# yeyupiaoling/MASR

Measured on AMD Instinct MI355X. Metric: audio-seconds/sec (RTF^-1), conformer_streaming_fbank b32x10s, PCM->fbank->encoder->ctc_greedy->text, higher is better.
Workload: dtype f32; 1 GPU; configs[1]: conformer.yml streaming fbank, batch=32 synthetic 16 kHz 10 s utterances per GPU, ctc_greedy, random-init weights V=4233; global_batch=32, parallelism=dp1, world_size_observed=1, backend=none

## Files before the change

### masr_amd/_lib.py

```python
import collections
import contextlib
import ctypes as C
import os

import numpy as _np

from .build import LIB_PATH

_lib = None


class MasrConfig(C.Structure):
    _fields_ = [('model_kind', C.c_int32), ('d_model', C.c_int32), ('heads', C.c_int32), ('d_ff', C.c_int32),
                ('num_blocks', C.c_int32), ('cnn_kernel', C.c_int32), ('n_mels', C.c_int32),
                ('vocab_size', C.c_int32), ('causal', C.c_int32), ('max_pos', C.c_int32), ('device_id', C.c_int32),
                ('reserved', C.c_int32 * 5)]


class MasrError(RuntimeError):
    pass


_P = C.c_void_p
_I = C.c_int32
# ... 115 lines not shown

def lib():
    global _lib
    if _lib is not None:
        return _lib
    import torch
    if not os.path.exists(LIB_PATH):
        raise MasrError(f'{LIB_PATH} not found: build it with `python -m masr_amd.build` '
                        f'(hipcc --offload-arch=gfx950). There is no CPU fallback.')
    h = C.CDLL(LIB_PATH)
    for name, args in SIGNATURES.items():
        fn = getattr(h, name)
        fn.argtypes = args
        fn.restype = _RESTYPE.get(name, C.c_int)
    _lib = h
    return h


def check(rc):
    if rc != 0:
        raise MasrError(lib().masr_last_error().decode('utf-8', 'replace'))


_ENGINE_KEYS = {'beam_profile': 2, 'prof_stride': 16, 'skip_padding': 38}


def debug_key_table():
    rows = []
    key, default, experimental, name = _I(), _I(), _I(), C.c_char_p()
    while lib().masr_debug_key_info(len(rows), C.byref(key), C.byref(default), C.byref(experimental), C.byref(name)) == 0:
        rows.append((key.value, name.value.decode(), default.value, bool(experimental.value)))
    return rows


FFN_KERNELS = ('X3', 'COOP', 'DUAL', 'ROWS16', 'PC')
FfnPlan = collections.namedtuple('FfnPlan', 'kernel nsplit cpb ny packed tail_in_kernel head_in_kernel split_head prof')


def ffn_plan(d_ff, M, keys=None, d_model=256, affine=0, tail_n=0, tail_planar=0, head_ktaps=0, head_norm=0):
    ask = (_I * 5)(affine, tail_n, tail_planar, head_ktaps, head_norm)
    flat = [int(v) for kv in (keys or {}).items() for v in kv]
    out = (_I * 9)()
    check(lib().masr_ffn_plan(d_model, d_ff, M, ask, (_I * max(1, len(flat)))(*flat), len(flat) // 2, out))
    return FfnPlan(FFN_KERNELS[out[0]], *out[1:])


@contextlib.contextmanager
# ... 11 lines not shown
```

### masr_amd/csrc/common.h

```cpp
#pragma once
#include <hip/hip_runtime.h>
#include <stdint.h>

#include "knobs.h"
#include "lm_scorer.h"

struct masr_resample_feed;
struct masr_resample_rate;

#ifndef MASR_EXPERIMENTS
#define MASR_EXPERIMENTS 0
#endif

typedef float f32x4 __attribute__((ext_vector_type(4)));
typedef float f32x16 __attribute__((ext_vector_type(16)));

namespace masr {

struct LdsAttr {
    size_t granted[32] = {};
};
void ensure_dynamic_lds(const void* fn, size_t bytes, LdsAttr& st);
void note_launch_error(const char* what, hipError_t e);

// ... 87 lines not shown
    const float *feats, *mean, *istd, *c1w, *c1b;
    int Tin, Fin;
};

void launch_gemm(const GemmArgs& a, int amode, int epi, hipStream_t s);
void launch_pack_conv2_rows(const float* w, float* p, int K, hipStream_t s);
bool gemm_conv2_rows(const GemmArgs& a);
void launch_gemm_splitk(const GemmArgs& a, float* partial, int nsplit, hipStream_t s, int amode = A_PLAIN);
struct FfnArgs;
#if MASR_EXPERIMENTS
bool launch_gemm_bf16x3(const GemmArgs& a, int amode, hipStream_t s);
size_t ffn_x3_packed_elems(int dff);
void launch_pack_ffn_x3(const float* w1, const float* w2, unsigned short* p1, unsigned short* p2, int dff, hipStream_t s);
bool launch_ffn_x3(const FfnArgs& a, hipStream_t s);
#else
inline bool launch_gemm_bf16x3(const GemmArgs&, int, hipStream_t) { return false; }
inline size_t ffn_x3_packed_elems(int) { return 0; }
inline void launch_pack_ffn_x3(const float*, const float*, unsigned short*, unsigned short*, int, hipStream_t) {}
inline bool launch_ffn_x3(const FfnArgs&, hipStream_t) { return false; }
#endif

void launch_layernorm(const float* x, const float* w, const float* b, float* y, int M, float eps,
                      int seq_t, int pad, const int* lens, hipStream_t s);
void launch_conv1(const float* feats, const float* mean, const float* istd, const float* w9c, const float* bias,
                  float* out, int B, int T, int F, int C, hipStream_t s);
bool launch_dwconv_ln_silu(const float* g, const float* wkc, const float* bias, const float* lnw, const float* lnb,
                           float* out, int nseq, int Tq, int ktaps, float eps, hipStream_t s, const float* gconst = nullptr);
void launch_glu_const(const float* bias512, float* out256, hipStream_t s);
void launch_queue_spin(long long ticks, hipStream_t s);
void launch_queue_nop(hipStream_t s);
bool launch_dwconv_bn_silu(const float* g, const float* wkc, const float* bias, const float* scale, const float* shift,
                           float* out, int nseq, int Tq, int ktaps, hipStream_t s, const float* gconst = nullptr);
void launch_dwconv_stride2_ln_silu(const float* g, const float* wkc, const float* bias, const float* lnw,
                                   const float* lnb, float* out, int nseq, int Tin, int ktaps, float eps, hipStream_t s);
void launch_dwconv_stride2_bn_silu(const float* g, const float* wkc, const float* bias, const float* scale,
                                   const float* shift, float* out, int nseq, int Tin, int ktaps, hipStream_t s);
void launch_avgpool2(const float* x, float* out, int B, int T, hipStream_t s);
void launch_time_reduce_dw(const float* x, const float* w5c, const float* bias, const int* lens, float* out, int B, int T,
                           int mstride, hipStream_t s);
void launch_recover_add(const float* saved, const float* y, float* x, int B, int T, int L, hipStream_t s);
void launch_softmax_argmax(float* logits, int M, int V, int ldv, int write_probs, int* idx, float* maxp, hipStream_t s);
void launch_ctc_collapse(const int* idx, const float* maxp, const int* nframes, int B, int Tp, int blank,
                         int* tokens, int* ntok, float* score, hipStream_t s);
struct PoolSeg {
    long src, dst;
    int n, pad_;
// ... 32 lines not shown
    float* C;
    const float* R;
    float* R2;
    const int* lens;
    int* out_idx;
    float* out_maxp;
    int M, N;
    int lda, ldc, ldr;
    float eps, alpha;
    int seq_t, pad;
    int mask_tp;
    int mstride;
    int out_seq_t;
    int out_pad_l, out_pad_tot;
    int plane_cols;
    long plane_stride;
    int a_seq_t, a_seq_stride;
    float* const* cache_rd;
    float* const* cache_wr;
    int hist_affine;
    const float* dw_w;
    const float* dw_b;
    const float* gconst;
    const AttSeq* kv_seqs;
    int kv_tq;
};
bool launch_rowgemm(const RowGemmArgs& a, int pro, int epi, hipStream_t s);
bool launch_rowgemm_small(const RowGemmArgs& a, int pro, int epi, hipStream_t s);

struct FfnPostLn {
    const float* lnw;
    const float* lnb;
    float* y;
    float eps = 1e-5f;
};
struct FfnTail {
    const float* lnw;
    const float* lnb;
    const float* W;
    const float* bias;
    float* out;
    int N, ldo;
    const float* pre_lnw;
    const float* pre_lnb;
    long plane_stride;
    int seq_t, pad_t;
// ... 159 lines not shown
    float eps;
};
#if MASR_EXPERIMENTS
bool launch_attn_chain(const AttnChainArgs& a, int max_nq, hipStream_t s);
#else
inline bool launch_attn_chain(const AttnChainArgs&, int, hipStream_t) { return false; }
#endif
enum PosEnc { POS_ENC_REL = 0, POS_ENC_ABS = 1, POS_ENC_NONE = 2 };
enum AttPos { ATT_REL_POS = 0, ATT_NO_POS = 1 };
void launch_attention(const AttSeq* seqs, int nseq, int max_nq, int heads, int q_stride, int kv_stride,
                      const float* ptab , const float* bias_u, const float* bias_v,
                      int chunk_size, int pos_stride, hipStream_t s, int row_w, int pos_mode);
void launch_add_pos_rows(float* x, const float* pe, const int* offs, int nseq, int Tq, int d, int n_pos, hipStream_t s);
void launch_attention_grouped(const AttSeq* seqs, int nseq, int max_nq, int heads, int group, const float* ptab,
                              int t_true, const float* bias_u, const float* bias_v, hipStream_t s, int chunk_size = 0);
void launch_attseq_grouped(AttSeq* seqs, const float* q, const float* k, const float* v, float* out, const int* lens,
                           int B, int Tg, int group, int mstride, hipStream_t s);
void launch_kv_append(const AttSeq* seqs, const float* qkv, int n, int Tq, hipStream_t s);
void launch_cnn_cache_move(float* const* caches, float* lnpad, int n, int Tq, int pad, int dir, hipStream_t s);
void launch_conv_hist(const float* x, const float* w, const float* b, float* const* cache_rd, float* const* cache_wr,
                      float* lnpad, int n, int Tq, int pad, int affine, float eps, hipStream_t s);
void launch_attseq_full(AttSeq* seqs, const float* qkv, float* out, const int* lens, int B, int Tp, int mstride,
                        hipStream_t s, int valid_only = 0);

bool wide_supported(int d);
bool launch_layernorm_wide(const float* x, const float* w, const float* b, float* y, int M, int d, float eps, int seq_t, int pad,
                           const int* lens, hipStream_t s);
void launch_conv1_wide(const float* feats, const float* mean, const float* istd, const float* w9c, const float* bias, float* out,
                       int B, int T, int F, int C, hipStream_t s);
bool launch_glu_wide(const float* in, float* out, int M, int d, hipStream_t s);
void launch_glu_const_wide(const float* bias2d, float* out, int d, hipStream_t s);
bool launch_dwconv_ln_silu_wide(const float* g, const float* wkc, const float* bias, const float* lnw, const float* lnb, float* out,
                                int nseq, int Tq, int d, int ktaps, int in_pad, int pad_l, float eps, const float* gconst, int act,
                                hipStream_t s);
bool launch_conv_hist_wide(const float* x, const float* w, const float* b, float* const* cache_rd, float* const* cache_wr,
                           float* lnpad, int n, int Tq, int pad, int d, float eps, hipStream_t s);
bool launch_kv_append_wide(const AttSeq* seqs, const float* qkv, int n, int Tq, int d, hipStream_t s);
void launch_attseq_full_wide(AttSeq* seqs, const float* qkv, float* out, const int* lens, int B, int Tp, int d, hipStream_t s);

void launch_dec_embed(const int* hyp, const int* lens, const float* emb, const float* pe, float* x, int S, int Lmax, int d, int V,
                      int reverse, hipStream_t s);
void launch_dec_attention(const float* q, int q_stride, const float* k, const float* v, int kv_stride, float* out, int out_stride,
                          const int* hyp_lens, const int* key_lens, int S, int N, int Lmax, int Tp, int heads, int causal,
                          hipStream_t s);
void launch_dec_scores(const float* logits, const int* hyp, const int* lens, float* rowlp, float* out, int S, int Lmax, int V,
                       int reverse, hipStream_t s);
// ... 24 lines not shown
```

### masr_amd/csrc/elementwise.hip

```cpp
#include <algorithm>

#include "common.h"

namespace masr {

__device__ __forceinline__ float wave_sum(float v) {
    return wave_sum_dpp(v);
}
__device__ __forceinline__ float wave_max(float v) {
#pragma unroll
    for (int o = 32; o > 0; o >>= 1) v = fmaxf(v, __shfl_xor(v, o, 64));
    return v;
}

__global__ __launch_bounds__(256) void layernorm256_kernel(const float* __restrict__ x, const float* __restrict__ w,
                                                           const float* __restrict__ b, float* y, int M, float eps,
                                                           int seq_t, int pad, const int* __restrict__ lens) {
    const int lane = threadIdx.x & 63;
    const int row = blockIdx.x * 4 + (threadIdx.x >> 6);
    if (row >= M) return;
    size_t orow = row;
    bool zero = false;
    if (seq_t > 0) {
        const int bb = row / seq_t, t = row - bb * seq_t;
// ... 3 lines not shown
    f32x4 o;
    if (zero) {
        o = f32x4{0.f, 0.f, 0.f, 0.f};
    } else {
        const f32x4 v = *reinterpret_cast<const f32x4*>(x + (size_t)row * 256 + lane * 4);
        const float mean = wave_sum(v[0] + v[1] + v[2] + v[3]) * (1.0f / 256.0f);
        const float d0 = v[0] - mean, d1 = v[1] - mean, d2 = v[2] - mean, d3 = v[3] - mean;
        const float var = wave_sum(d0 * d0 + d1 * d1 + d2 * d2 + d3 * d3) * (1.0f / 256.0f);
        const float rstd = 1.0f / sqrtf(var + eps);
        const f32x4 ww = *reinterpret_cast<const f32x4*>(w + lane * 4);
        const f32x4 bb = *reinterpret_cast<const f32x4*>(b + lane * 4);
        o[0] = d0 * rstd * ww[0] + bb[0];
        o[1] = d1 * rstd * ww[1] + bb[1];
        o[2] = d2 * rstd * ww[2] + bb[2];
        o[3] = d3 * rstd * ww[3] + bb[3];
    }
    *reinterpret_cast<f32x4*>(y + orow * 256 + lane * 4) = o;
}

void launch_layernorm(const float* x, const float* w, const float* b, float* y, int M, float eps, int seq_t, int pad,
                      const int* lens, hipStream_t s) {
    if (M <= 0) return;
    hipLaunchKernelGGL(layernorm256_kernel, dim3((M + 3) / 4), dim3(256), 0, s, x, w, b, y, M, eps, seq_t, pad, lens);
}

__global__ __launch_bounds__(256) void affine_rows_kernel(const float* __restrict__ x, const float* __restrict__ w,
                                                          const float* __restrict__ b, float* y, int M, int seq_t, int pad) {
    const int lane = threadIdx.x & 63;
    const int row = blockIdx.x * 4 + (threadIdx.x >> 6);
    if (row >= M) return;
    const int bb = row / seq_t, t = row - bb * seq_t;
    const size_t orow = (size_t)bb * (seq_t + pad) + pad + t;
    const f32x4 v = *reinterpret_cast<const f32x4*>(x + (size_t)row * 256 + lane * 4);
    const f32x4 ww = *reinterpret_cast<const f32x4*>(w + lane * 4);
    const f32x4 bv = *reinterpret_cast<const f32x4*>(b + lane * 4);
    f32x4 o;
#pragma unroll
    for (int i = 0; i < 4; ++i) o[i] = ww[i] * v[i] + bv[i];
    *reinterpret_cast<f32x4*>(y + orow * 256 + lane * 4) = o;
}
void launch_affine_rows(const float* x, const float* w, const float* b, float* y, int M, int seq_t, int pad, hipStream_t s) {
    if (M <= 0) return;
    hipLaunchKernelGGL(affine_rows_kernel, dim3((M + 3) / 4), dim3(256), 0, s, x, w, b, y, M, seq_t, pad);
}

template <int NT>
// ... 525 lines not shown

void launch_argmax_rows(const float* probs, int M, int V, int* idx, float* maxp, hipStream_t s) {
    if (M <= 0) return;
    hipLaunchKernelGGL(argmax_rows_kernel, dim3(M), dim3(256), 0, s, probs, V, idx, maxp);
}

__global__ void frame_counts_kernel(const int* __restrict__ nsamp, int B, int* nfr, int* nenc, int halve, int il) {
    const int b = blockIdx.x * blockDim.x + threadIdx.x;
    if (b >= B) return;
    const int n = nsamp[b];
    const int T = n >= 400 ? 1 + (n - 400) / 160 : 0;
    if (nfr) nfr[b] = T;
    if (nenc) {
        const int n4 = sub_frames(il, T);
        nenc[b] = halve ? (n4 + 1) / 2 : n4;
    }
}

void launch_frame_counts(const int* nsamp, int B, int* nfr, int* nenc, int halve, hipStream_t s, int input_layer) {
    if (B <= 0) return;
    hipLaunchKernelGGL(frame_counts_kernel, dim3((B + 63) / 64), dim3(64), 0, s, nsamp, B, nfr, nenc, halve, input_layer);
}

__global__ void sub_lens_kernel(const int* __restrict__ lens, int B, int rate, int* __restrict__ out) {
    const int b = blockIdx.x * blockDim.x + threadIdx.x;
    if (b < B) out[b] = 4 * ((max(lens[b], 0) + rate - 1) / rate);
}
void launch_sub_lens(const int* lens, int B, int rate, int* out, hipStream_t s) {
    if (B <= 0) return;
    hipLaunchKernelGGL(sub_lens_kernel, dim3((B + 63) / 64), dim3(64), 0, s, lens, B, rate, out);
}

__global__ __launch_bounds__(256) void add_pos_rows_kernel(float* __restrict__ x, const float* __restrict__ pe,
                                                           const int* __restrict__ offs, int nseq, int Tq, int d4, int n_pos) {
    const int i = blockIdx.x * 256 + threadIdx.x;
    if (i >= nseq * Tq * d4) return;
    const int row = i / d4, c = i - row * d4;
    const int b = row / Tq, t = row - b * Tq;
    const int p = (offs ? offs[b] : 0) + t;
    if (p < 0 || p >= n_pos) return;
    f32x4 v = reinterpret_cast<f32x4*>(x)[i];
    const f32x4 q = reinterpret_cast<const f32x4*>(pe)[(size_t)p * d4 + c];
    v[0] += q[0]; v[1] += q[1]; v[2] += q[2]; v[3] += q[3];
    reinterpret_cast<f32x4*>(x)[i] = v;
}
void launch_add_pos_rows(float* x, const float* pe, const int* offs, int nseq, int Tq, int d, int n_pos, hipStream_t s) {
// ... 223 lines not shown
```

### masr_amd/csrc/engine.hip

```cpp
#include <math.h>
#include <stdio.h>
#include <stdlib.h>
#include <string.h>

#include <map>
#include <mutex>
#include <string>
#include <vector>

#include "../../include/masr_hip.h"
#include "common.h"
#include "ffn_plan.h"

using namespace masr;
namespace masr {
int lm_device_view(masr_lm* lm, LmView* out);
bool lm_word_based(const masr_lm* lm);
}
extern "C" const char* masr_lm_last_error(void);

static thread_local std::string g_err;
static int fail(const std::string& m) {
    g_err = m;
    return 1;
// ... 226 lines not shown

struct masr_engine : EngineWs {
    masr_config cfg;
    DecoderState dec;
    EngineWs parked[MASR_LANES];
    int lane = 0;
    hipEvent_t pack_ev = nullptr;
    void* pack_stream = nullptr;
    bool pack_pending = false;
    bool finalized = false;
    std::map<std::string, HostTensor> host;
    std::vector<void*> owned;
    float *cmvn_mean = nullptr, *cmvn_istd = nullptr, *conv1_w = nullptr, *conv1_b = nullptr, *conv2_w = nullptr,
          *conv2_b = nullptr, *conv3_w = nullptr, *conv3_b = nullptr, *embed_w = nullptr, *embed_b = nullptr, *after_w = nullptr, *after_b = nullptr,
          *ctc_w = nullptr, *ctc_b = nullptr, *pe = nullptr;
    std::vector<LayerW> layers;
    std::vector<SqLayerW> sq_layers;
    std::vector<Ds2LayerW> ds2_layers;
    std::vector<GBeam> gbeams;
    DevBuf beam_pool, beam_state;
    std::map<void*, std::pair<DevBuf, DevBuf>> beam_ws;
    std::map<void*, DevBuf> ms_ws;
    int skip_padding = 7;
    void* beam_first_stream = nullptr;
    bool beam_first_set = false;
    std::map<std::pair<int, const float*>, PackedW> packed;
    long long* beam_prof = nullptr;
    float *preln_w = nullptr, *preln_b = nullptr, *tr_dw_w = nullptr, *tr_dw_b = nullptr, *tr_pw_w = nullptr,
          *tr_pw_b = nullptr, *rec_w = nullptr, *rec_b = nullptr;
    int reduce_idx = -1, recover_idx = -1;
    int stride_idx = -1, n_group_layers = 0, group_size = 3;
    int input_layer = IL_CONV2D;
    bool conv_bn = false;
    bool ds2_gru = false;
    int pos_enc = POS_ENC_REL;
    int act = ENC_ACT_SWISH;
    float *window = nullptr, *melwt = nullptr, *tw512 = nullptr, *twr4 = nullptr;
    FbankTables fbank_tables() const { return FbankTables{window, melwt, tw512, twr4, mel_lo}; }
    int* mel_lo = nullptr;
    float *dct = nullptr, *lifter = nullptr;
    int dct_ceps = 0;
    double *lin_win = nullptr, *lin_tw = nullptr;
    double lin_scale = 0.0;
    std::vector<Stream> streams;
    int prof_kind = 0;
    int prof_stride = 1, prof_seen = 0;
// ... 1617 lines not shown
                float* hn = hbuf + (size_t)((step + 1) & 1) * hsz;
                const int miss = gru ? launch_gru_step(e->gx.as<float>(), w.whh, w.bhn, hp, hn, e->rnn_out.as<float>(), xl, nseq, Tq, H, step, ndir, s)
                                     : launch_lstm_step(e->gx.as<float>(), w.whh, hp, hn, cbuf, e->rnn_out.as<float>(), xl, nseq, Tq, H, step, ndir, s);
                if (miss) return fail("deepspeech2: no recurrent step kernel for rnn_size=" + std::to_string(H));
            }
        }
        if (st) {
            const float* hfin = hbuf + (size_t)(Tq & 1) * hsz;
            for (int i = 0; i < nseq; ++i) {
                float* hc = st[i]->cnn.as<float>() + (size_t)l * 2 * H;
                HIPCHK(hipMemcpyAsync(hc, hfin + (size_t)i * H, sizeof(float) * H, hipMemcpyDeviceToDevice, s));
                HIPCHK(hipMemcpyAsync(hc + H, (gru ? hfin : cbuf) + (size_t)i * H, sizeof(float) * H, hipMemcpyDeviceToDevice, s));
            }
        }
        float* out = l == L - 1 ? enc_out : e->ln.as<float>();
        launch_layernorm_generic(e->rnn_out.as<float>(), w.ln_w, w.ln_b, out, M, D, 1e-5f, s);
        in = out;
    }
    LAUNCHCHK();
    if (Tq_out) *Tq_out = Tq;
    return 0;
}

extern "C" {

int masr_encode_full(masr_engine* e, const float* feats_dev, const int32_t* feat_lens_dev, int32_t B, int32_t T,
                     int32_t decoding_chunk_size, float* enc_out_dev, void* stream) {
    if (!e || !e->finalized) return fail("engine not finalized");
    ENTER(e);
    CallGuard call_guard(e, (hipStream_t)stream);
    if (B <= 0) return fail("empty batch");
    hipStream_t s = (hipStream_t)stream;
    if (e->cfg.model_kind == 3) return ds2_forward(e, s, feats_dev, feat_lens_dev, B, T, enc_out_dev, nullptr, nullptr);
    const int chunk = (decoding_chunk_size > 0 && e->cfg.causal) ? decoding_chunk_size : 0;
    if (feat_lens_dev && e->input_layer != IL_CONV2D && !(feat_lens_dev = sub_lens(e, s, feat_lens_dev, B)))
        return fail("out of device memory (subsampled lengths)");
    if (e->cfg.model_kind == 1) return encode_full_squeezeformer(e, s, feats_dev, feat_lens_dev, B, T, enc_out_dev, chunk);
    if (e->cfg.model_kind == 2) return encode_full_efficient(e, s, feats_dev, feat_lens_dev, B, T, enc_out_dev, chunk);
    if (is_wide(e)) return encode_full_wide(e, s, feats_dev, feat_lens_dev, B, T, enc_out_dev, chunk);
    const int d = e->cfg.d_model, H = e->cfg.heads, pad = e->cfg.cnn_kernel - 1;
    int Tq = 0;
    CHK(embed(e, s, feats_dev, B, T, &Tq));
    if (Tq >= e->cfg.max_pos) return fail("sequence longer than max_pos");
    add_abs_pos(e, s, B, Tq, nullptr);
    const int M = B * Tq;
    CHK(ensure_layer_ws(e, B, Tq));
    CHK(e->attseq.ensure(sizeof(AttSeq) * B));
    float* x = e->x.as<float>();
    EncodeCtx ctx{B, Tq, feat_lens_dev};
    launch_attseq_full(e->attseq.as<AttSeq>(), e->qkv.as<float>(), e->att.as<float>(), feat_lens_dev, B, Tq, 4, s);
    if (!e->cfg.causal)
        HIPCHK(hipMemsetAsync(e->glu.p, 0, (size_t)B * (Tq + pad) * d * sizeof(float), s));
    const LayerW* prev = nullptr;
    const bool few_rows = few_row_blocks(knobs(), M);
    for (const LayerW& w : e->layers) {
        FfnArgs f1 = ffn_macaron(w, M);
        f1.tail = qkv_tail(e, w, e->qkv.as<float>(), 3 * d);
        if (prev) { f1.tail.pre_lnw = prev->ln_fin_w; f1.tail.pre_lnb = prev->ln_fin_b; }
        const FfnDone r1 = ffn(e, s, f1);
        CHK(r1);
        if (!r1.tail_done) mhsa(e, s, w, M);
        const bool fuse_ac = knobs().attn_chain && !few_rows && !knobs().no_chain && H == 4 && d == 256 && knobs().rowgemm_packed &&
                             e->pos_enc == POS_ENC_REL;
        if (fuse_ac) {
            AttnChainArgs a{};
            a.seqs = e->attseq.as<AttSeq>(); a.nseq = B; a.q_stride = 3 * d; a.kv_stride = 3 * d;
            a.chunk_size = (decoding_chunk_size > 0 && e->cfg.causal) ? decoding_chunk_size : 0; a.pos_stride = 1;
            a.ptab = w.ptab; a.bias_u = w.pos_u; a.bias_v = w.pos_v;
            a.Wp = packed_rows_of(e, w.chain_w, 3 * d, s); a.bias = w.chain_b; a.lnw = w.ln_conv_w; a.lnb = w.ln_conv_b;
            a.R = x; a.R2 = x; a.C = e->glu.as<float>(); a.lens = feat_lens_dev; a.seq_t = Tq; a.mstride = 4;
            a.out_pad_l = e->cfg.causal ? pad : pad / 2; a.out_pad_tot = pad; a.eps = 1e-5f;
            if (!a.Wp) return fail("packed chain weights: allocation failed");
            ProfScope ps(e, s, PROF_ATT, 6.0 * d * (double)Tq * Tq * B + 2.0 * M * (double)(3 * d) * d);
            launch_attn_chain(a, Tq, s);
        } else {
// ... 1 lines not shown
            launch_attention(e->attseq.as<AttSeq>(), B, Tq, H, 3 * d, 3 * d, w.ptab, w.pos_u, w.pos_v,
                             (decoding_chunk_size > 0 && e->cfg.causal) ? decoding_chunk_size : 0, 1, s, 256, att_pos(e));
        }
        if (few_rows) {
            mhsa_out(e, s, w, M);
            const bool fuse = knobs().split_head && e->cfg.cnn_kernel == 15 && knobs().ffn_packed >= 2 && !knobs().no_ffn_head;
            CHK(conv_module(e, s, w, ctx, false, 0, 4, false, fuse));
            FfnArgs f2 = ffn_final(w, M, x);
            if (fuse) f2.head = conv_head(e, w, feat_lens_dev, Tq, e->cfg.cnn_kernel, 4);
            CHK(ffn(e, s, f2));
            continue;
        } else if (knobs().no_chain) {
            mhsa_out(e, s, w, M);
            CHK(conv_module(e, s, w, ctx, false));
            CHK(ffn(e, s, ffn_final(w, M)));
        } else {
            if (!fuse_ac) mhsa_out_pw1(e, s, w, ctx);
            FfnArgs f2 = ffn_final(w, M);
            f2.head = conv_head(e, w, feat_lens_dev, Tq, e->cfg.cnn_kernel, 4);
            CHK(ffn(e, s, f2));
        }
        prev = &w;
    }
    if (prev) launch_layernorm(x, prev->ln_fin_w, prev->ln_fin_b, x, M, 1e-5f, 0, 0, nullptr, s);
    launch_layernorm(x, e->after_w, e->after_b, enc_out_dev, M, 1e-5f, 0, 0, nullptr, s);
    LAUNCHCHK();
    return 0;
}

static int ctc_head(masr_engine* e, const float* enc_dev, int M, float* probs_dev, int write_probs, int32_t* argmax_dev,
                    float* maxprob_dev, hipStream_t s) {
    const int d = enc_dim(e), V = e->cfg.vocab_size;
    float* logits = probs_dev;
    if (!logits) {
        CHK(e->logits.ensure((size_t)M * V * sizeof(float)));
        logits = e->logits.as<float>();
    }
    gemm(e, s, enc_dev, d, e->ctc_w, e->ctc_b, logits, V, M, V, d, ACT_NONE, 1.f, nullptr, 0);
    launch_softmax_argmax(logits, M, V, V, write_probs, argmax_dev, maxprob_dev, s);
    LAUNCHCHK();
    return 0;
}

int masr_ctc_probs(masr_engine* e, const float* enc_dev, int32_t M, float* probs_dev, int32_t* argmax_dev,
                   float* maxprob_dev, void* stream) {
    if (!e || !e->finalized) return fail("engine not finalized");
    ENTER(e);
    CallGuard call_guard(e, (hipStream_t)stream);
    if (!probs_dev) return fail("probs_dev is null");
    if (e->cfg.vocab_size > 16384) return fail("vocab_size > 16384 is not supported by the softmax / pruning kernels (one 256-thread workgroup holds a row in registers)");
    return ctc_head(e, enc_dev, M, probs_dev, 1, argmax_dev, maxprob_dev, (hipStream_t)stream);
// ... 214 lines not shown
    gbeam_args(*g, a);
    CHK(bind_lm(a, g->lm, g->alpha, g->beta));
    a.init = g->started ? 0 : 1;
    a.prof = nullptr;
    a.tokens = tokens_dev; a.len = len_dev; a.score = score_dev;
    if (launch_beam_search(a, 1, (hipStream_t)stream)) return fail("beam search launch rejected the sizes");
    LAUNCHCHK();
    g->started = true;
    return 0;
}

int masr_fbank_batch(masr_engine* e, const void* samples_dev, int32_t sample_format, const int32_t* n_samples_dev,
                     int32_t B, int32_t n_max, int32_t use_db_normalization, float target_db, float* feats_dev,
                     int32_t* n_frames_dev, int16_t* norm_pcm_dev, float* gain_dev, void* stream) {
    if (!e) return fail("null engine");
    ENTER(e);
    if (sample_format != 0 && sample_format != 1) return fail("sample_format must be 0 (int16) or 1 (float32)");
    hipStream_t s = (hipStream_t)stream;
    const int T_max = n_max >= 400 ? 1 + (n_max - 400) / 160 : 0;
    CHK(e->gain.ensure(sizeof(float) * fbank_gain_scratch_floats(B)));
    float* gain = e->gain.as<float>();
    if (use_db_normalization == 2) {
        if (!gain_dev) return fail("use_db_normalization = 2 needs the gains in gain_dev");
        HIPCHK(hipMemcpyAsync(gain, gain_dev, sizeof(float) * B, hipMemcpyDeviceToDevice, s));
    }
    {
        ProfScope ps(e, s, PROF_FBANK, 0.0);
        launch_fbank(samples_dev, sample_format, n_samples_dev, B, n_max, use_db_normalization, target_db, e->fbank_tables(),
                     feats_dev, T_max, gain, norm_pcm_dev, s);
    }
    if (gain_dev && use_db_normalization == 1)
        HIPCHK(hipMemcpyAsync(gain_dev, gain, sizeof(float) * B, hipMemcpyDeviceToDevice, s));
    if (n_frames_dev) launch_frame_counts(n_samples_dev, B, n_frames_dev, nullptr, 0, s);
    LAUNCHCHK();
    return 0;
}

int masr_mean_square(masr_engine* e, const void* samples_dev, int32_t sample_format, const int32_t* n_samples_dev, int32_t B,
                     int32_t n_max, float* mean_square_dev, void* stream) {
    if (!e || !mean_square_dev) return fail("null argument");
    ENTER(e);
    if (sample_format != 0 && sample_format != 1) return fail("sample_format must be 0 (int16) or 1 (float32)");
    DevBuf& ws = e->ms_ws[stream];
    CHK(ws.ensure(sizeof(float) * fbank_gain_scratch_floats(B)));
    launch_mean_square(samples_dev, sample_format, n_samples_dev, B, n_max, ws.as<float>(), mean_square_dev,
                       (hipStream_t)stream);
    LAUNCHCHK();
// ... 133 lines not shown
                           int32_t n_max, int32_t use_db_normalization, float target_db, const float* gain_dev,
                           int32_t decode_all_frames, int32_t* tokens_dev, int32_t* n_tokens_dev, float* score_dev,
                           int32_t* rows_dev, void* stream) {
    if (!e || !e->finalized) return fail("engine not finalized");
    ENTER(e);
    CallGuard call_guard(e, (hipStream_t)stream);
    if (n_max < 400) return fail("n_max < 400 samples: no frame");
    hipStream_t s = (hipStream_t)stream;
    const int d = enc_dim(e), F = e->cfg.n_mels;
    const int T = 1 + (n_max - 400) / 160, Tsub = sub_frames(e->input_layer, T);
    const bool halved = e->cfg.model_kind == 2 && e->stride_idx >= 0;
    const int Tq = halved ? (Tsub + 1) / 2 : Tsub;
    if (Tsub <= 0) return fail("utterances too short");
    CHK(e->feats.ensure((size_t)B * T * F * sizeof(float)));
    CHK(e->nframes.ensure(sizeof(int) * 2 * B));
    CHK(e->enc.ensure((size_t)B * Tq * d * sizeof(float)));
    CHK(e->idx.ensure(sizeof(int) * B * Tq));
    CHK(e->maxp.ensure(sizeof(float) * B * Tq));
    int* nfr = e->nframes.as<int>();
    int* nenc = nfr + B;
    CHK(masr_fbank_batch(e, samples_dev, fmt, n_samples_dev, B, n_max, use_db_normalization, target_db,
                         e->feats.as<float>(), nullptr, nullptr, use_db_normalization == 2 ? const_cast<float*>(gain_dev) : nullptr,
                         stream));
    launch_frame_counts(n_samples_dev, B, nfr, nenc, halved ? 1 : 0, s, e->input_layer);
    {
        const int keep = e->skip_padding;
        if (decode_all_frames) e->skip_padding = 0;
        const int rc = masr_encode_full(e, e->feats.as<float>(), nfr, B, T, -1, e->enc.as<float>(), stream);
        e->skip_padding = keep;
        if (rc) return rc;
    }
    CHK(masr_ctc_greedy_frames(e, e->enc.as<float>(), B * Tq, e->idx.as<int>(), e->maxp.as<float>(), stream));
    if (rows_dev) {
        launch_ctc_collapse_rows(e->idx.as<int>(), e->maxp.as<float>(), decode_all_frames ? nullptr : nenc, B, Tq, 0, rows_dev, s);
        LAUNCHCHK();
        return 0;
    }
    CHK(masr_ctc_collapse(e, e->idx.as<int>(), e->maxp.as<float>(), decode_all_frames ? nullptr : nenc, B, Tq, 0,
                          tokens_dev, n_tokens_dev, score_dev, stream));
    return 0;
}

int masr_transcribe_batch(masr_engine* e, const int16_t* pcm_dev, const int32_t* n_samples_dev, int32_t B,
                          int32_t n_max, int32_t use_db_normalization, float target_db, int32_t decode_all_frames,
                          int32_t* tokens_dev, int32_t* n_tokens_dev, float* score_dev, void* stream) {
    if (use_db_normalization == 2) return fail("masr_transcribe_batch: supplied gains go through masr_transcribe_rows");
    return transcribe_impl(e, pcm_dev, 0, n_samples_dev, B, n_max, use_db_normalization, target_db, nullptr, decode_all_frames,
                           tokens_dev, n_tokens_dev, score_dev, nullptr, stream);
}

int masr_transcribe_rows(masr_engine* e, const void* samples_dev, int32_t sample_format, const int32_t* n_samples_dev, int32_t B,
                         int32_t n_max, int32_t use_db_normalization, float target_db, const float* gain_dev,
                         int32_t decode_all_frames, int32_t* rows_dev, void* stream) {
    if (!rows_dev) return fail("null argument");
    if (sample_format != 0 && sample_format != 1) return fail("sample_format: 0 = int16 PCM, 1 = float32");
// ... 710 lines not shown
    e->parked[lane] = EngineWs();
    e->lane = lane;
    return 0;
}

int masr_side_stream(masr_engine* e, int32_t kind, void** stream_out) {
    if (!e || !stream_out) return fail("null argument");
    if (kind < 0 || kind >= MASR_SIDE_STREAMS)
        return fail("masr_side_stream: kind must be 0 / 1 (prefix search), 2 (preparation), 3 (copy) or 4 (second encoder lane)");
    SideStreams* ss = nullptr;
    if (side_streams_of(e->cfg.device_id, &ss)) return 1;
    *stream_out = (void*)ss->s[kind];
    return 0;
}

int masr_debug_set(masr_engine* e, int32_t key, int32_t value) {
    if (!e) return fail("null engine");
    const KnobInfo* k = knob_find(key);
    if (k) {
        if (!MASR_EXPERIMENTS && k->experimental && value != 0)
            return fail("masr_debug_set: this key selects an experimental kernel that is not in this build (MASR_BUILD_EXPERIMENTS=1)");
        knob_set(key, value);
    } else if (key == 38) e->skip_padding = value;
    else if (key == 16) { e->prof_stride = value > 1 ? value : 1; e->prof_seen = 0; }
    else if (key == 2) {
        if (value) {
            if (!e->beam_prof) {
                void* p = nullptr;
                HIPCHK(hipMalloc(&p, 16 * sizeof(long long)));
                e->owned.push_back(p);
                e->beam_prof = (long long*)p;
            }
        } else if (e->beam_prof) {
            long long h[16];
            HIPCHK(hipMemcpy(h, e->beam_prof, sizeof(h), hipMemcpyDeviceToHost));
            fprintf(stderr, "beam phases (cycles, last workgroup): setup+hash %lld  extensions %lld  prefixes+count %lld  select %lld  compact %lld\n",
                    h[0], h[1], h[2], h[3], h[4]);
            fprintf(stderr, "  narrow step (%lld frames): tables+candidates %lld  hash+contexts %lld  children+scorer table %lld  extensions %lld  "
                    "prefixes+select %lld  scan %lld  survivors %lld  new prefixes %lld\n", h[5], h[6], h[7], h[8], h[9], h[10], h[11], h[12], h[13]);
            if (h[15] > 0) fprintf(stderr, "  wide step (%lld frames): %.1f distinct scorer contexts per frame\n", h[15], (double)h[14] / (double)h[15]);
            e->beam_prof = nullptr;
        }
    }
    else return fail("unknown debug key");
    return 0;
}

int masr_debug_reset(masr_engine* e) {
    if (!e) return fail("null engine");
    knobs_reset();
    e->skip_padding = 7;
    e->prof_stride = 1;
    e->prof_seen = 0;
    return 0;
}

int masr_debug_key_info(int32_t index, int32_t* key, int32_t* default_value, int32_t* experimental, const char** name) {
    const KnobInfo* k = knob_info(index);
    if (!k) return 1;
    if (key) *key = k->key;
    if (default_value) *default_value = knob_default(*k);
    if (experimental) *experimental = k->experimental;
    if (name) *name = k->name;
    return 0;
}

int masr_ffn_plan(int32_t d_model, int32_t d_ff, int32_t m, const int32_t* ask, const int32_t* overrides, int32_t n_overrides,
                  int32_t* plan) {
    if (!ask || !plan || n_overrides < 0 || (n_overrides && !overrides)) return fail("masr_ffn_plan: null argument");
    if (d_ff <= 0 || d_ff % 128 || m <= 0) return fail("masr_ffn_plan: d_ff must be a positive multiple of 128 and m positive");
    Knobs k;
    for (int i = 0; i < n_overrides; ++i)
        if (!knob_set(overrides[2 * i], overrides[2 * i + 1], k))
            return fail("masr_ffn_plan: no process-wide switch has key " + std::to_string(overrides[2 * i]));
// ... 290 lines not shown
```

### masr_amd/csrc/rowgemm.hip

```cpp
#include <cstdio>
#include <cstdlib>

#include "common.h"

namespace masr {

static constexpr int RG_BM = 32;
static constexpr int RG_K = 256;
static constexpr int RG_ALD = RG_K + 4;
static constexpr int RG_WLD = 32 + 4;
static constexpr int RG_WSLAB = 32 * RG_WLD;
static constexpr int RG_NSET = 4;

__device__ __forceinline__ float rg_wsum(float v) {
    return wave_sum_dpp(v);
}

template <int PRO, int EPI, int GSPLIT, int PACKED = 0>
__global__ __launch_bounds__(512) void rowgemm_kernel(RowGemmArgs p) {
    extern __shared__ __align__(16) float sm[];
    float* at = sm;
    float* wpv = at + RG_BM * RG_ALD;
    float* red = wpv + 8 * 2 * RG_WSLAB;

// ... 16 lines not shown
            const int row = row0 + wave * 4 + rr;
            bool live = row < p.M;
            size_t src_row = live ? row : 0;
            if (PRO == RG_PRO_PLAIN && p.a_seq_t > 0) {
                const int rc = live ? row : 0;
                const int b = rc / p.a_seq_t;
                src_row = (size_t)b * p.a_seq_stride + (rc - b * p.a_seq_t);
            }
            if (PRO == RG_PRO_AFFINE && p.lens && p.seq_t > 0) {
                const int rc = live ? row : 0;
                const int b = rc / p.seq_t, t = rc - b * p.seq_t;
                live = live && p.mstride * t < p.lens[b];
            }
            if (PRO == RG_PRO_LN_PAD) {
                const int per = p.seq_t + p.pad;
                const int rc = live ? row : 0;
                const int b = rc / per, tp = rc - b * per;
                const int t = max(tp - p.pad, 0);
                live = live && tp >= p.pad && !(p.lens && p.mstride * t >= p.lens[b]);
                src_row = (size_t)b * p.seq_t + t;
            }
            live4[rr] = live;
            v4[rr] = *reinterpret_cast<const f32x4*>(p.A + src_row * p.lda + lane * 4);
        }
#pragma unroll
        for (int rr = 0; rr < 4; ++rr) {
            const int lr = wave * 4 + rr;
            const f32x4 v = v4[rr];
            f32x4 o;
            if (PRO == RG_PRO_PLAIN) {
                o = v;
            } else if (PRO == RG_PRO_AFFINE) {
                o[0] = gw[0] * v[0] + gb[0];
                o[1] = gw[1] * v[1] + gb[1];
                o[2] = gw[2] * v[2] + gb[2];
                o[3] = gw[3] * v[3] + gb[3];
            } else {
                const float mean = rg_wsum(v[0] + v[1] + v[2] + v[3]) * (1.0f / 256.0f);
                const float d0 = v[0] - mean, d1 = v[1] - mean, d2 = v[2] - mean, d3 = v[3] - mean;
                const float var = rg_wsum(d0 * d0 + d1 * d1 + d2 * d2 + d3 * d3) * (1.0f / 256.0f);
                const float rstd = 1.0f / sqrtf(var + p.eps);
                o[0] = d0 * rstd * gw[0] + gb[0];
                o[1] = d1 * rstd * gw[1] + gb[1];
                o[2] = d2 * rstd * gw[2] + gb[2];
                o[3] = d3 * rstd * gw[3] + gb[3];
            }
// ... 333 lines not shown
```

Before: 53100 audio-seconds/sec.

## Fuse encode setup, pad zeroing, final layernorms into CTC head, drop gain copy

Adds a single encode-setup kernel that computes frame counts, builds the attention sequence descriptors and zeroes only the GLU pad rows instead of memsetting the whole buffer. The two trailing layernorms are fused into one kernel, or folded into the CTC rowgemm prologue when the CTC head is used. The gain buffer is used directly rather than copied. Each change targets small launch and memory-traffic overheads, and each sits behind a new debug key that defaults to on. The deferred-LN path depends on the rowgemm LN prologue being the right one for the CTC epilogue.

```diff
diff --git a/masr_amd/_lib.py b/masr_amd/_lib.py
--- a/masr_amd/_lib.py
+++ b/masr_amd/_lib.py
@@ -161,7 +161,8 @@
         raise MasrError(lib().masr_last_error().decode('utf-8', 'replace'))
 
 
-_ENGINE_KEYS = {'beam_profile': 2, 'prof_stride': 16, 'skip_padding': 38}
+_ENGINE_KEYS = {'beam_profile': 2, 'prof_stride': 16, 'skip_padding': 38, 'encode_setup': 45, 'glu_pad_zero': 46, 'gain_direct': 47,
+                'final_ln_fused': 48}
 
 
 def debug_key_table():
diff --git a/masr_amd/csrc/common.h b/masr_amd/csrc/common.h
--- a/masr_amd/csrc/common.h
+++ b/masr_amd/csrc/common.h
@@ -133,6 +133,8 @@
 
 void launch_layernorm(const float* x, const float* w, const float* b, float* y, int M, float eps,
                       int seq_t, int pad, const int* lens, hipStream_t s);
+void launch_layernorm2(const float* x, const float* w1, const float* b1, const float* w2, const float* b2, float* y, int M, float eps,
+                       hipStream_t s);
 void launch_conv1(const float* feats, const float* mean, const float* istd, const float* w9c, const float* bias,
                   float* out, int B, int T, int F, int C, hipStream_t s);
 bool launch_dwconv_ln_silu(const float* g, const float* wkc, const float* bias, const float* lnw, const float* lnb,
@@ -211,6 +213,8 @@
     const float* dw_w;
     const float* dw_b;
     const float* gconst;
+    const float* pre_lnw;
+    const float* pre_lnb;
     const AttSeq* kv_seqs;
     int kv_tq;
 };
@@ -416,6 +420,20 @@
                       float* lnpad, int n, int Tq, int pad, int affine, float eps, hipStream_t s);
 void launch_attseq_full(AttSeq* seqs, const float* qkv, float* out, const int* lens, int B, int Tp, int mstride,
                         hipStream_t s, int valid_only = 0);
+struct EncodeSetupArgs {
+    const int* nsamp;
+    int* nfr;
+    int* nenc;
+    int halve, il;
+    const int* lens;
+    AttSeq* seqs;
+    const float* qkv;
+    float* out;
+    int B, Tp, mstride;
+    float* glu;
+    int pad_l, pad_tot;
+};
+void launch_encode_setup(const EncodeSetupArgs& a, hipStream_t s);
 
 bool wide_supported(int d);
 bool launch_layernorm_wide(const float* x, const float* w, const float* b, float* y, int M, int d, float eps, int seq_t, int pad,
diff --git a/masr_amd/csrc/elementwise.hip b/masr_amd/csrc/elementwise.hip
--- a/masr_amd/csrc/elementwise.hip
+++ b/masr_amd/csrc/elementwise.hip
@@ -49,6 +49,47 @@
                       const int* lens, hipStream_t s) {
     if (M <= 0) return;
     hipLaunchKernelGGL(layernorm256_kernel, dim3((M + 3) / 4), dim3(256), 0, s, x, w, b, y, M, eps, seq_t, pad, lens);
+}
+
+__global__ __launch_bounds__(256) void layernorm256x2_kernel(const float* __restrict__ x, const float* __restrict__ w1,
+                                                             const float* __restrict__ b1, const float* __restrict__ w2,
+                                                             const float* __restrict__ b2, float* y, int M, float eps) {
+    const int lane = threadIdx.x & 63;
+    const int row = blockIdx.x * 4 + (threadIdx.x >> 6);
+    if (row >= M) return;
+    f32x4 v = *reinterpret_cast<const f32x4*>(x + (size_t)row * 256 + lane * 4);
+    {
+        const float mean = wave_sum(v[0] + v[1] + v[2] + v[3]) * (1.0f / 256.0f);
+        const float d0 = v[0] - mean, d1 = v[1] - mean, d2 = v[2] - mean, d3 = v[3] - mean;
+        const float var = wave_sum(d0 * d0 + d1 * d1 + d2 * d2 + d3 * d3) * (1.0f / 256.0f);
+        const float rstd = 1.0f / sqrtf(var + eps);
+        const f32x4 ww = *reinterpret_cast<const f32x4*>(w1 + lane * 4);
+        const f32x4 bb = *reinterpret_cast<const f32x4*>(b1 + lane * 4);
+        v[0] = d0 * rstd * ww[0] + bb[0];
+        v[1] = d1 * rstd * ww[1] + bb[1];
+        v[2] = d2 * rstd * ww[2] + bb[2];
+        v[3] = d3 * rstd * ww[3] + bb[3];
+    }
+    f32x4 o;
+    {
+        const float mean = wave_sum(v[0] + v[1] + v[2] + v[3]) * (1.0f / 256.0f);
+        const float d0 = v[0] - mean, d1 = v[1] - mean, d2 = v[2] - mean, d3 = v[3] - mean;
+        const float var = wave_sum(d0 * d0 + d1 * d1 + d2 * d2 + d3 * d3) * (1.0f / 256.0f);
+        const float rstd = 1.0f / sqrtf(var + eps);
+        const f32x4 ww = *reinterpret_cast<const f32x4*>(w2 + lane * 4);
+        const f32x4 bb = *reinterpret_cast<const f32x4*>(b2 + lane * 4);
+        o[0] = d0 * rstd * ww[0] + bb[0];
+        o[1] = d1 * rstd * ww[1] + bb[1];
+        o[2] = d2 * rstd * ww[2] + bb[2];
+        o[3] = d3 * rstd * ww[3] + bb[3];
+    }
+    *reinterpret_cast<f32x4*>(y + (size_t)row * 256 + lane * 4) = o;
+}
+
+void launch_layernorm2(const float* x, const float* w1, const float* b1, const float* w2, const float* b2, float* y, int M, float eps,
+                       hipStream_t s) {
+    if (M <= 0) return;
+    hipLaunchKernelGGL(layernorm256x2_kernel, dim3((M + 3) / 4), dim3(256), 0, s, x, w1, b1, w2, b2, y, M, eps);
 }
 
 __global__ __launch_bounds__(256) void affine_rows_kernel(const float* __restrict__ x, const float* __restrict__ w,
@@ -620,6 +661,50 @@
     hipLaunchKernelGGL(frame_counts_kernel, dim3((B + 63) / 64), dim3(64), 0, s, nsamp, B, nfr, nenc, halve, input_layer);
 }
 
+__global__ __launch_bounds__(256) void encode_setup_kernel(EncodeSetupArgs a) {
+    if (blockIdx.x == 0 && a.seqs) {
+        for (int b = threadIdx.x; b < a.B; b += 256) {
+            int len;
+            if (a.nsamp) {
+                const int n = a.nsamp[b];
+                const int T = n >= 400 ? 1 + (n - 400) / 160 : 0;
+                a.nfr[b] = T;
+                const int n4 = sub_frames(a.il, T);
+                a.nenc[b] = a.halve ? (n4 + 1) / 2 : n4;
+                len = T;
+            } else {
+                len = a.lens[b];
+            }
+            AttSeq s;
+            s.q = a.qkv + (size_t)b * a.Tp * 768;
+            s.k = s.q + 256;
+            s.v = s.q + 512;
+            s.out = a.out + (size_t)b * a.Tp * 256;
+            s.nq = a.Tp;
+            s.nk = a.Tp;
+            s.klen = min(a.Tp, (len + a.mstride - 1) / a.mstride);
+            s.pos0 = 0;
+            s.q_abs0 = 0;
+            s.pad_ = 0;
+            a.seqs[b] = s;
+        }
+    }
+    if (!a.glu) return;
+    const int per = a.pad_tot * 64;
+    const int total = a.B * per;
+    for (int i = blockIdx.x * 256 + threadIdx.x; i < total; i += gridDim.x * 256) {
+        const int b = i / per, r = (i - b * per) >> 6, c4 = i & 63;
+        const size_t row = (size_t)b * (a.Tp + a.pad_tot) + (r < a.pad_l ? r : a.Tp + r);
+        *reinterpret_cast<f32x4*>(a.glu + row * 256 + c4 * 4) = f32x4{0.f, 0.f, 0.f, 0.f};
+    }
+}
+
+void launch_encode_setup(const EncodeSetupArgs& a, hipStream_t s) {
+    if (a.B <= 0) return;
+    const int blocks = a.glu ? std::max(1, std::min(256, (a.B * a.pad_tot * 64 + 255) / 256)) : 1;
+    hipLaunchKernelGGL(encode_setup_kernel, dim3(blocks), dim3(256), 0, s, a);
+}
+
 __global__ void sub_lens_kernel(const int* __restrict__ lens, int B, int rate, int* __restrict__ out) {
     const int b = blockIdx.x * blockDim.x + threadIdx.x;
     if (b < B) out[b] = 4 * ((max(lens[b], 0) + rate - 1) / rate);
diff --git a/masr_amd/csrc/engine.hip b/masr_amd/csrc/engine.hip
--- a/masr_amd/csrc/engine.hip
+++ b/masr_amd/csrc/engine.hip
@@ -272,6 +272,10 @@
     std::map<void*, std::pair<DevBuf, DevBuf>> beam_ws;
     std::map<void*, DevBuf> ms_ws;
     int skip_padding = 7;
+    int encode_setup = 1;
+    int glu_pad_zero = 1;
+    int gain_direct = 1;
+    int final_ln_fused = 1;
     void* beam_first_stream = nullptr;
     bool beam_first_set = false;
     std::map<std::pair<int, const float*>, PackedW> packed;
@@ -1935,15 +1939,41 @@
     return 0;
 }
 
+namespace {
+struct EncodeExtras {
+    const int* nsamp = nullptr;
+    int* nfr = nullptr;
+    int* nenc = nullptr;
+    int halve = 0;
+    bool may_defer_ln = false;
+    bool deferred = false;
+    const float* pre_lnw = nullptr;
+    const float* pre_lnb = nullptr;
+};
+int encode_full_impl(masr_engine* e, const float* feats_dev, const int32_t* feat_lens_dev, int32_t B, int32_t T,
+                     int32_t decoding_chunk_size, float* enc_out_dev, void* stream, EncodeExtras* ex);
+}
+
 extern "C" {
 
 int masr_encode_full(masr_engine* e, const float* feats_dev, const int32_t* feat_lens_dev, int32_t B, int32_t T,
                      int32_t decoding_chunk_size, float* enc_out_dev, void* stream) {
+    return encode_full_impl(e, feats_dev, feat_lens_dev, B, T, decoding_chunk_size, enc_out_dev, stream, nullptr);
+}
+
+}
+
+namespace {
+
+int encode_full_impl(masr_engine* e, const float* feats_dev, const int32_t* feat_lens_dev, int32_t B, int32_t T,
+                     int32_t decoding_chunk_size, float* enc_out_dev, void* stream, EncodeExtras* ex) {
     if (!e || !e->finalized) return fail("engine not finalized");
     ENTER(e);
     CallGuard call_guard(e, (hipStream_t)stream);
     if (B <= 0) return fail("empty batch");
     hipStream_t s = (hipStream_t)stream;
+    const bool setup_counts = ex && ex->nsamp && e->encode_setup && e->cfg.model_kind == 0 && !is_wide(e) && e->input_layer == IL_CONV2D;
+    if (ex && ex->nsamp && !setup_counts) launch_frame_counts(ex->nsamp, B, ex->nfr, ex->nenc, ex->halve, s, e->input_layer);
     if (e->cfg.model_kind == 3) return ds2_forward(e, s, feats_dev, feat_lens_dev, B, T, enc_out_dev, nullptr, nullptr);
     const int chunk = (decoding_chunk_size > 0 && e->cfg.causal) ? decoding_chunk_size : 0;
     if (feat_lens_dev && e->input_layer != IL_CONV2D && !(feat_lens_dev = sub_lens(e, s, feat_lens_dev, B)))
@@ -1961,9 +1991,25 @@
     CHK(e->attseq.ensure(sizeof(AttSeq) * B));
     float* x = e->x.as<float>();
     EncodeCtx ctx{B, Tq, feat_lens_dev};
-    launch_attseq_full(e->attseq.as<AttSeq>(), e->qkv.as<float>(), e->att.as<float>(), feat_lens_dev, B, Tq, 4, s);
-    if (!e->cfg.causal)
-        HIPCHK(hipMemsetAsync(e->glu.p, 0, (size_t)B * (Tq + pad) * d * sizeof(float), s));
+    {
+        const bool pad_rows = !e->cfg.causal && pad > 0 && e->glu_pad_zero;
+        EncodeSetupArgs a{};
+        a.lens = feat_lens_dev; a.seqs = e->attseq.as<AttSeq>(); a.qkv = e->qkv.as<float>(); a.out = e->att.as<float>();
+        a.B = B; a.Tp = Tq; a.mstride = 4; a.il = e->input_layer;
+        if (setup_counts) { a.nsamp = ex->nsamp; a.nfr = ex->nfr; a.nenc = ex->nenc; a.halve = ex->halve; }
+        if (pad_rows) { a.glu = e->glu.as<float>(); a.pad_l = pad / 2; a.pad_tot = pad; }
+        if (e->encode_setup) {
+            launch_encode_setup(a, s);
+        } else {
+            launch_attseq_full(a.seqs, a.qkv, a.out, feat_lens_dev, B, Tq, 4, s);
+            if (pad_rows) {
+                EncodeSetupArgs z{};
+                z.B = B; z.Tp = Tq; z.glu = a.glu; z.pad_l = a.pad_l; z.pad_tot = a.pad_tot;
+                launch_encode_setup(z, s);
+            }
+        }
+        if (!e->cfg.causal && !pad_rows) HIPCHK(hipMemsetAsync(e->glu.p, 0, (size_t)B * (Tq + pad) * d * sizeof(float), s));
+    }
     const LayerW* prev = nullptr;
     const bool few_rows = few_row_blocks(knobs(), M);
     for (const LayerW& w : e->layers) {
@@ -2011,11 +2057,23 @@
         }
         prev = &w;
     }
-    if (prev) launch_layernorm(x, prev->ln_fin_w, prev->ln_fin_b, x, M, 1e-5f, 0, 0, nullptr, s);
-    launch_layernorm(x, e->after_w, e->after_b, enc_out_dev, M, 1e-5f, 0, 0, nullptr, s);
+    if (ex && ex->may_defer_ln) {
+        ex->deferred = true;
+        ex->pre_lnw = prev ? prev->ln_fin_w : nullptr;
+        ex->pre_lnb = prev ? prev->ln_fin_b : nullptr;
+    } else if (prev && e->final_ln_fused) {
+        launch_layernorm2(x, prev->ln_fin_w, prev->ln_fin_b, e->after_w, e->after_b, enc_out_dev, M, 1e-5f, s);
+    } else {
+        if (prev) launch_layernorm(x, prev->ln_fin_w, prev->ln_fin_b, x, M, 1e-5f, 0, 0, nullptr, s);
+        launch_layernorm(x, e->after_w, e->after_b, enc_out_dev, M, 1e-5f, 0, 0, nullptr, s);
+    }
     LAUNCHCHK();
     return 0;
 }
+
+}
+
+extern "C" {
 
 static int ctc_head(masr_engine* e, const float* enc_dev, int M, float* probs_dev, int write_probs, int32_t* argmax_dev,
                     float* maxprob_dev, hipStream_t s) {
@@ -2276,7 +2334,8 @@
     float* gain = e->gain.as<float>();
     if (use_db_normalization == 2) {
         if (!gain_dev) return fail("use_db_normalization = 2 needs the gains in gain_dev");
-        HIPCHK(hipMemcpyAsync(gain, gain_dev, sizeof(float) * B, hipMemcpyDeviceToDevice, s));
+        if (e->gain_direct) gain = gain_dev;
+        else HIPCHK(hipMemcpyAsync(gain, gain_dev, sizeof(float) * B, hipMemcpyDeviceToDevice, s));
     }
     {
         ProfScope ps(e, s, PROF_FBANK, 0.0);
@@ -2456,15 +2515,25 @@
     CHK(masr_fbank_batch(e, samples_dev, fmt, n_samples_dev, B, n_max, use_db_normalization, target_db,
                          e->feats.as<float>(), nullptr, nullptr, use_db_normalization == 2 ? const_cast<float*>(gain_dev) : nullptr,
                          stream));
-    launch_frame_counts(n_samples_dev, B, nfr, nenc, halved ? 1 : 0, s, e->input_layer);
+    EncodeExtras ex;
+    ex.nsamp = n_samples_dev; ex.nfr = nfr; ex.nenc = nenc; ex.halve = halved ? 1 : 0;
+    ex.may_defer_ln = e->final_ln_fused && e->cfg.model_kind == 0 && !is_wide(e) && (B * Tq + 31) / 32 >= knobs().ctc_fused_blocks;
     {
         const int keep = e->skip_padding;
         if (decode_all_frames) e->skip_padding = 0;
-        const int rc = masr_encode_full(e, e->feats.as<float>(), nfr, B, T, -1, e->enc.as<float>(), stream);
+        const int rc = encode_full_impl(e, e->feats.as<float>(), nfr, B, T, -1, e->enc.as<float>(), stream, &ex);
         e->skip_padding = keep;
         if (rc) return rc;
     }
-    CHK(masr_ctc_greedy_frames(e, e->enc.as<float>(), B * Tq, e->idx.as<int>(), e->maxp.as<float>(), stream));
+    if (ex.deferred) {
+        RowGemmArgs g = rg_args(e->x.as<float>(), e->cfg.d_model, e->ctc_w, e->ctc_b, nullptr, 0, B * Tq, e->cfg.vocab_size);
+        g.lnw = e->after_w; g.lnb = e->after_b; g.pre_lnw = ex.pre_lnw; g.pre_lnb = ex.pre_lnb;
+        g.out_idx = e->idx.as<int>(); g.out_maxp = e->maxp.as<float>();
+        rowgemm(e, s, RG_PRO_LN, RG_EPI_CTC, g);
+        LAUNCHCHK();
+    } else {
+        CHK(masr_ctc_greedy_frames(e, e->enc.as<float>(), B * Tq, e->idx.as<int>(), e->maxp.as<float>(), stream));
+    }
     if (rows_dev) {
         launch_ctc_collapse_rows(e->idx.as<int>(), e->maxp.as<float>(), decode_all_frames ? nullptr : nenc, B, Tq, 0, rows_dev, s);
         LAUNCHCHK();
@@ -3221,6 +3290,10 @@
             return fail("masr_debug_set: this key selects an experimental kernel that is not in this build (MASR_BUILD_EXPERIMENTS=1)");
         knob_set(key, value);
     } else if (key == 38) e->skip_padding = value;
+    else if (key == 45) e->encode_setup = value;
+    else if (key == 46) e->glu_pad_zero = value;
+    else if (key == 47) e->gain_direct = value;
+    else if (key == 48) e->final_ln_fused = value;
     else if (key == 16) { e->prof_stride = value > 1 ? value : 1; e->prof_seen = 0; }
     else if (key == 2) {
         if (value) {
@@ -3249,6 +3322,7 @@
     if (!e) return fail("null engine");
     knobs_reset();
     e->skip_padding = 7;
+    e->encode_setup = e->glu_pad_zero = e->gain_direct = e->final_ln_fused = 1;
     e->prof_stride = 1;
     e->prof_seen = 0;
     return 0;
diff --git a/masr_amd/csrc/rowgemm.hip b/masr_amd/csrc/rowgemm.hip
--- a/masr_amd/csrc/rowgemm.hip
+++ b/masr_amd/csrc/rowgemm.hip
@@ -62,6 +62,24 @@
             }
             live4[rr] = live;
             v4[rr] = *reinterpret_cast<const f32x4*>(p.A + src_row * p.lda + lane * 4);
+        }
+        if (PRO == RG_PRO_LN && EPI == RG_EPI_CTC && p.pre_lnw) {
+            const f32x4 pw = *reinterpret_cast<const f32x4*>(p.pre_lnw + lane * 4);
+            const f32x4 pb = *reinterpret_cast<const f32x4*>(p.pre_lnb + lane * 4);
+#pragma unroll
+            for (int rr = 0; rr < 4; ++rr) {
+                const f32x4 v = v4[rr];
+                const float mean = rg_wsum(v[0] + v[1] + v[2] + v[3]) * (1.0f / 256.0f);
+                const float d0 = v[0] - mean, d1 = v[1] - mean, d2 = v[2] - mean, d3 = v[3] - mean;
+                const float var = rg_wsum(d0 * d0 + d1 * d1 + d2 * d2 + d3 * d3) * (1.0f / 256.0f);
+                const float rstd = 1.0f / sqrtf(var + p.eps);
+                f32x4 o;
+                o[0] = d0 * rstd * pw[0] + pb[0];
+                o[1] = d1 * rstd * pw[1] + pb[1];
+                o[2] = d2 * rstd * pw[2] + pb[2];
+                o[3] = d3 * rstd * pw[3] + pb[3];
+                v4[rr] = o;
+            }
         }
 #pragma unroll
         for (int rr = 0; rr < 4; ++rr) {
```

Measured after the change: 52980 audio-seconds/sec. About the same (-0.2%).
